# TuragaLab/flybody

Measured on AMD Instinct MI355X. Metric: env steps/sec (whole node), walk_imitation 4096-batch random-action rollout, higher is better.
Workload: dtype f64

## Files before the change

### flybody_amd/csrc/fb_constraint.hpp

```cpp
#pragma once
#include "fb_types.hpp"
#include "fb_math.hpp"
#include "fb_smooth.hpp"
#include "fb_newton.hpp"

#define JIDX(side, s, r) (((r)*2 + (side))*FB_MAXCH + (s))
#define MINIMP ((real)0.0001)
#define MAXIMP ((real)0.9999)

template <typename real>
FBD real get_impedance(const real* si, real pos, real margin) {
  real s0 = fmin(MAXIMP, fmax(MINIMP, si[0])), s1 = fmin(MAXIMP, fmax(MINIMP, si[1]));
  real s2 = fmax((real)0, si[2]), s3 = fmin(MAXIMP, fmax(MINIMP, si[3])), s4 = fmax((real)1, si[4]);
  if (s0 == s1 || s2 <= FB_MINV) return (real)0.5*(s0 + s1);
  real x = fabs((pos - margin)/s2);
  if (x >= 1) return s1;
  if (x <= 0) return s0;
  real y;
  if (s4 == 1) y = x;
  else if (s4 == 2) y = (x <= s3) ? x*x/s3 : 1 - (1 - x)*(1 - x)/(1 - s3);
  else if (x <= s3) y = pow(x, s4) / pow(s3, s4 - 1);
  else y = 1 - pow(1 - x, s4) / pow(1 - s3, s4 - 1);
  return s0 + y*(s1 - s0);
}
// ... 120 lines not shown
        real jp[3] = {0, 0, 0};
        const FB_LDS real* cp = w.lLD + 6*((sl < len) ? dof : 0);
        real cd[6];
#pragma unroll
        for (int k = 0; k < 6; k++) cd[k] = cp[k];
        if (sl < len) {
          real tt[3]; cross3(tt, cd, off);
          jp[0] = cd[3] + tt[0]; jp[1] = cd[4] + tt[1]; jp[2] = cd[5] + tt[2];
        }
        const real sgn = side ? (real)1 : (real)-1;
        for (int k = 0; k < cdim; k++) w.efc_J()[JIDX(side, sl, cadr + k)] = sgn*dot3(fr + 3*k, jp);
      }
    }
  }
  if (lane == 0) {
    if (nefc > w.istate()[IS_MAX_NEFC]) w.istate()[IS_MAX_NEFC] = nefc;
    if (nefc > 32) w.istate()[IS_N_GT32]++;
    if (nefc > 64) w.istate()[IS_N_GT64]++;
    w.istate()[IS_NEFC] = nefc; w.istate()[IS_NLIMIT] = nlimit; if (ob || nlimit > FB_MAXEFC_) { atomicOr(w.istate() + IS_WARN, (int)WARN_EFC_CAP); atomicOr(w.istate() + IS_WARN_EVER, (int)WARN_EFC_CAP); } }
  SYNC();
}

#define ARIDX(r, c) ((r)*((r) + 1)/2 + (c))

template <typename real, typename ARP>
FB_STAGE_B void d_build_AR(const DevModel<real>& M, const WS<real>& w, ARP AR, int nefc, int lane);

template <typename real>
FBD void project_row(const DevModel<real>& M, const WS<real>& w, int side, int r, int body, int len, const FB_LDS real* sd, real* y) {
  int chain[FB_MAXCH], rowadr[FB_MAXCH];
  load_chain(M, body, chain);
#pragma unroll
  for (int s = 0; s < FB_MAXCH; s++) { y[s] = (s < len) ? w.efc_J()[JIDX(side, s, r)] : (real)0; rowadr[s] = (int)w.lmadr()[chain[s]] + s; }
  const int chmax = M.chmax;
#pragma unroll
  for (int s = FB_MAXCH - 1; s >= 1; s--) {
    if (s < chmax) {
      const FB_LDS real* row = w.lLD + rowadr[s];
#pragma unroll
      for (int t = 0; t < s; t++) y[t] -= row[-t] * y[s];
    }
  }
#pragma unroll
  for (int s = 0; s < FB_MAXCH; s++) y[s] = (s < len) ? y[s]*sd[chain[s]] : (real)0;
}

template <int TRUNK, typename real, typename ARP>
FBD void ar_from_registers_t(const DevModel<real>& M, const WS<real>& w, ARP AR, int nefc, int lane, const real* yA, const real* yB, int bA, int bB, int lA, int lB) {
  const bool valid = lane < nefc;
  const int c = lane;
  const int* common = M.body_common; const int nb = M.nbody;
  int rbA = rdlane(bA, 0), rbB = rdlane(bB, 0);
  int cAA = common[rbA*nb + bA], cAB = common[rbA*nb + bB], cBA = common[rbB*nb + bA], cBB = common[rbB*nb + bB];
  const real Rc = valid ? w.efc_R()[c] : (real)0;
  real tr[TRUNK > 0 ? TRUNK : 1];
#pragma unroll
  for (int s = 0; s < TRUNK; s++) tr[s] = yA[s] + yB[s];
  for (int r = 0; r < nefc; r++) {
    int rlA = rdlane(lA, r), rlB = rdlane(lB, r);
    int cmAA = min(min(cAA, lA), rlA), cmAB = min(min(cAB, lB), rlA), cmBA = min(min(cBA, lA), rlB), cmBB = min(min(cBB, lB), rlB);
    if (r + 1 < nefc) {
      rbA = rdlane(bA, r + 1); rbB = rdlane(bB, r + 1);
      cAA = common[rbA*nb + bA]; cAB = common[rbA*nb + bB]; cBA = common[rbB*nb + bA]; cBB = common[rbB*nb + bB];
    }
    real acc = 0;
#pragma unroll
    for (int s = 0; s < TRUNK; s++) acc += rdlane(tr[s], r)*tr[s];
#pragma unroll
    for (int s0 = 0; s0 < FB_MAXCH; s0 += 4) {
      if (s0 + 4 > TRUNK && s0 < rlA) {
#pragma unroll
        for (int s = s0; s < s0 + 4; s++) if (s >= TRUNK) { real yr = rdlane(yA[s], r); if (s < cmAA) acc += yr*yA[s]; if (s < cmAB) acc += yr*yB[s]; }
      }
    }
#pragma unroll
    for (int s0 = 0; s0 < FB_MAXCH; s0 += 4) {
      if (s0 + 4 > TRUNK && s0 < rlB) {
#pragma unroll
        for (int s = s0; s < s0 + 4; s++) if (s >= TRUNK) { real yr = rdlane(yB[s], r); if (s < cmBA) acc += yr*yA[s]; if (s < cmBB) acc += yr*yB[s]; }
      }
    }
    if (valid && c <= r) {
      if (c == r) acc += Rc;
      AR[ARIDX(r, c)] = acc;
    }
  }
  SYNC();
}
template <int TRUNK, typename real, typename ARP>
FBD void ar_entry_lanes_t(const DevModel<real>& M, const WS<real>& w, ARP AR, int nefc, int lane, const real* yA, const real* yB, int bA, int bB, int lA, int lB) {
  const int* common = M.body_common; const int nb = M.nbody;
  const real Rl = w.efc_R()[lane];
  const int bodies = bA | (bB << 16), lens = lA | (lB << 8);
  real tr[TRUNK > 0 ? TRUNK : 1];
#pragma unroll
  for (int s = 0; s < TRUNK; s++) tr[s] = yA[s] + yB[s];
  unsigned any = 0;
#pragma unroll
  for (int g = 0; g < FB_MAXCH/4; g++) any |= (__ballot(lA > 4*g) != 0 ? 1u << g : 0u) | (__ballot(lB > 4*g) != 0 ? 0x100u << g : 0u);
  any = (unsigned)uniform_int((int)any);
  const int nent = nefc*(nefc + 1)/2;
  for (int p0 = 0; p0 < nent; p0 += FB_WAVE) {
    const int p = p0 + lane;
    const bool valid = p < nent;
    const int pp = valid ? p : 0;
    int r = (int)((sqrtf((float)(8*pp + 1)) - 1.0f)*0.5f);
    r -= (r*(r + 1)/2 > pp) ? 1 : 0;
    r += ((r + 1)*(r + 2)/2 <= pp) ? 1 : 0;
    const int c = pp - r*(r + 1)/2;
    const int rbod = nw_lane_i(bodies, r), cbod = nw_lane_i(bodies, c), rlen = nw_lane_i(lens, r), clen = nw_lane_i(lens, c);
    const int rbA = rbod & 0xffff, rbB = rbod >> 16, cbA = cbod & 0xffff, cbB = cbod >> 16;
    const int rlA = rlen & 0xff, rlB = rlen >> 8, clA = clen & 0xff, clB = clen >> 8;
    const int cmAA = min(min(common[rbA*nb + cbA], clA), rlA), cmAB = min(min(common[rbA*nb + cbB], clB), rlA);
    const int cmBA = min(min(common[rbB*nb + cbA], clA), rlB), cmBB = min(min(common[rbB*nb + cbB], clB), rlB);
    const real Rr = nw_lane(Rl, r);
    real acc = 0;
    {
      real tr_r[TRUNK > 0 ? TRUNK : 1], tr_c[TRUNK > 0 ? TRUNK : 1];
#pragma unroll
      for (int s = 0; s < TRUNK; s++) { tr_r[s] = nw_lane(tr[s], r); tr_c[s] = nw_lane(tr[s], c); }
#pragma unroll
      for (int s = 0; s < TRUNK; s++) acc += tr_r[s]*tr_c[s];
    }
#pragma unroll
    for (int s0 = 0; s0 < FB_MAXCH; s0 += 4) {
      if (s0 + 4 > TRUNK && ((any >> (s0/4)) & 1u)) {
        real yr[4], ya[4], yb[4];
#pragma unroll
        for (int s = s0; s < s0 + 4; s++) if (s >= TRUNK) { yr[s - s0] = nw_lane(yA[s], r); ya[s - s0] = nw_lane(yA[s], c); yb[s - s0] = nw_lane(yB[s], c); }
#pragma unroll
        for (int s = s0; s < s0 + 4; s++) if (s >= TRUNK) { if (s < cmAA) acc += yr[s - s0]*ya[s - s0]; if (s < cmAB) acc += yr[s - s0]*yb[s - s0]; }
      }
    }
#pragma unroll
    for (int s0 = 0; s0 < FB_MAXCH; s0 += 4) {
      if (s0 + 4 > TRUNK && ((any >> (8 + s0/4)) & 1u)) {
        real yr[4], ya[4], yb[4];
#pragma unroll
        for (int s = s0; s < s0 + 4; s++) if (s >= TRUNK) { yr[s - s0] = nw_lane(yB[s], r); ya[s - s0] = nw_lane(yA[s], c); yb[s - s0] = nw_lane(yB[s], c); }
#pragma unroll
        for (int s = s0; s < s0 + 4; s++) if (s >= TRUNK) { if (s < cmBA) acc += yr[s - s0]*ya[s - s0]; if (s < cmBB) acc += yr[s - s0]*yb[s - s0]; }
      }
    }
    if (valid) {
      if (c == r) acc += Rr;
      AR[p] = acc;
    }
  }
  SYNC();
}
template <typename real, typename ARP>
FBD void ar_from_registers(const DevModel<real>& M, const WS<real>& w, ARP AR, int nefc, int lane, const real* yA, const real* yB, int bA, int bB, int lA, int lB) {
  const bool entry = uniform_int(M.ar_entry_lanes) != 0;
  if (uniform_int(M.ntrunk) == FB_MAXTRUNK) {
    if (entry) ar_entry_lanes_t<FB_MAXTRUNK>(M, w, AR, nefc, lane, yA, yB, bA, bB, lA, lB);
    else ar_from_registers_t<FB_MAXTRUNK>(M, w, AR, nefc, lane, yA, yB, bA, bB, lA, lB);
  } else {
    if (entry) ar_entry_lanes_t<0>(M, w, AR, nefc, lane, yA, yB, bA, bB, lA, lB);
    else ar_from_registers_t<0>(M, w, AR, nefc, lane, yA, yB, bA, bB, lA, lB);
  }
}

template <typename real>
__device__ __forceinline__ void d_project_constraint(const DevModel<real>& M, const WS<real>& w, int lane) {
  int nefc = w.istate()[IS_NEFC];
  if (nefc == 0) return;
  FB_LDS real* sd = w.lx();
  for (int i = lane; i < M.nv; i += FB_WAVE) sd[i] = sqrt(w.lLD[w.lmadr()[i]]);
  SYNC();
  if (nefc <= FB_WAVE) {
    real yA[FB_MAXCH], yB[FB_MAXCH];
    int bA = 0, bB = 0, lA = 0, lB = 0;
    if (lane < nefc) { bA = w.efc_bA()[lane]; bB = w.efc_bB()[lane]; lA = w.efc_lA()[lane]; lB = w.efc_lB()[lane]; }
    project_row(M, w, 0, lane < nefc ? lane : 0, bA, lA, sd, yA);
    project_row(M, w, 1, lane < nefc ? lane : 0, bB, lB, sd, yB);
    if (nefc <= LdsCfg<real>::AR_ROWS) ar_from_registers(M, w, w.lAR(), nefc, lane, yA, yB, bA, bB, lA, lB);
    else ar_from_registers(M, w, w.AR(), nefc, lane, yA, yB, bA, bB, lA, lB);
    return;
  }
  for (int base = 0; base < nefc; base += FB_WAVE) {
    int r = base + lane;
    if (r < nefc) {
      for (int side = 0; side < 2; side++) {
        int body = side ? w.efc_bB()[r] : w.efc_bA()[r];
        int len = side ? w.efc_lB()[r] : w.efc_lA()[r];
        real y[FB_MAXCH];
        project_row(M, w, side, r, body, len, sd, y);
#pragma unroll
        for (int s = 0; s < FB_MAXCH; s++) w.efc_Y()[JIDX(side, s, r)] = y[s];
      }
    }
  }
  SYNC();
  const WS<real> wc = w;
  d_build_AR(M, wc, w.AR(), nefc, lane);
}

template <typename real, typename ARP>
FB_STAGE_B void d_build_AR(const DevModel<real>& M_, const WS<real>& w_, ARP AR, int nefc, int lane) {
  const DevModel<real>& M = as_constant(M_); const WS<real> w = ws_uniform(w_, M);
  for (int cbase = 0; cbase < nefc; cbase += FB_WAVE) {
    int c = cbase + lane;
    bool valid = c < nefc;
    real yA[FB_MAXCH], yB[FB_MAXCH];
    int bA = 0, bB = 0, lA = 0, lB = 0;
    if (valid) { bA = w.efc_bA()[c]; bB = w.efc_bB()[c]; lA = w.efc_lA()[c]; lB = w.efc_lB()[c]; }
#pragma unroll
    for (int s = 0; s < FB_MAXCH; s++) {
      yA[s] = valid ? w.efc_Y()[JIDX(0, s, c)] : (real)0;
      yB[s] = valid ? w.efc_Y()[JIDX(1, s, c)] : (real)0;
    }
    if (nefc <= FB_WAVE) {
      const int* common = M.body_common; const int nb = M.nbody;
      int rbA = rdlane(bA, 0), rbB = rdlane(bB, 0);
      int cAA = common[rbA*nb + bA], cAB = common[rbA*nb + bB], cBA = common[rbB*nb + bA], cBB = common[rbB*nb + bB];
      for (int r = 0; r < nefc; r++) {
        int rlA = rdlane(lA, r), rlB = rdlane(lB, r);
        int cmAA = min(min(cAA, lA), rlA), cmAB = min(min(cAB, lB), rlA), cmBA = min(min(cBA, lA), rlB), cmBB = min(min(cBB, lB), rlB);
        if (r + 1 < nefc) {
          rbA = rdlane(bA, r + 1); rbB = rdlane(bB, r + 1);
// ... 819 lines not shown
```

### flybody_amd/csrc/fb_engine.hip

```cpp
#ifdef FB_EMULATE
#include "emu/hip_emu.hpp"
#else
#include <hip/hip_runtime.h>
#endif
#include <algorithm>
#include <cmath>
#include <cstdio>
#include <cstdlib>
#include <cstring>
#include <map>
#include <stdexcept>
#include <string>
#include <vector>
#if defined(FB_EMULATE) && defined(FB_STATS)
extern "C" { long long fb_stats[64]; }
#endif

#include "../../include/flybody_engine.h"
#include "fb_step.hpp"
#include "fb_ik.hpp"
#include "fb_inverse.hpp"

static thread_local std::string g_err;
static int fail(const std::string& s) { g_err = s; return -1; }
// ... 853 lines not shown

static int alloc_obs(fb_batch* b, int nobs) {
  (void)hipFree(b->obs); b->obs = nullptr;
  HIPCHK(hipMalloc((void**)&b->obs, (size_t)b->n_env*nobs*sizeof(float)));
  HIPCHK(hipMemset(b->obs, 0, (size_t)b->n_env*nobs*sizeof(float)));
  b->nobs = nobs;
  return 0;
}

template <typename real>
static int build_devmodel(fb_batch* b, const fb_model* m, DevModel<real>& M) {
  memset(&M, 0, sizeof(M));
  M.nq = m->nq; M.nv = m->nv; M.nbody = m->nbody; M.njnt = m->njnt; M.ngeom = m->ngeom; M.nsite = m->nsite;
  M.nu = m->nu; M.na = m->na; M.ntendon = m->ntendon; M.npair = m->npair; M.nM = m->nM; M.nsubstep = m->nsubstep;
  M.nobsjnt = m->nobsjnt; M.napp = m->napp; M.nforce = m->nforce; M.ntouch = m->ntouch;
  M.site_thorax = m->i("sensor_site_thorax")[0]; M.nadh = (int)m->adh_act.size();
  M.iterations = m->i("opt_iterations")[0]; M.noslip_iterations = m->i("opt_noslip_iterations")[0];
  M.solver = (m->has("opt_solver", 1) && m->i("opt_solver")[0] == FB_SOLVER_PGS) ? FB_SOLVER_PGS : FB_SOLVER_NEWTON;
  M.timestep = (real)m->d("opt_timestep")[0]; M.control_timestep = (real)m->d("opt_control_timestep")[0];
  for (int k = 0; k < 3; k++) M.grav[k] = (real)m->d("opt_gravity")[k];
  M.density = (real)m->d("opt_density")[0]; M.viscosity = (real)m->d("opt_viscosity")[0];
  M.impratio = (real)m->d("opt_impratio")[0]; M.tolerance = (real)m->d("opt_tolerance")[0];
  {
    std::vector<double> rb; const double* r_ = m->d("geom_rbound");
    for (int g = 0; g < m->ngeom; g++) if (r_[g] > 0) rb.push_back(r_[g]);
    std::sort(rb.begin(), rb.end());
    M.vl_delta = (rb.empty() || m->npair <= 4*FB_WAVE) ? (real)0 : (real)(FB_VL_SCALE*rb[rb.size()/2]);
    { const char* e_ = getenv("FB_NO_NEIGHBOUR_LIST"); if (e_ && e_[0] == '1') M.vl_delta = 0; }
  }
  M.ar_entry_lanes = 1;
  { const char* e_ = getenv("FB_NO_AR_ENTRY_LANES"); if (e_ && e_[0] == '1') M.ar_entry_lanes = 0; }
  M.solver_handover = 1;
  { const char* e_ = getenv("FB_NO_SOLVER_HANDOVER"); if (e_ && e_[0] == '1') M.solver_handover = 0; }
  M.noslip_tolerance = (real)m->d("opt_noslip_tolerance")[0]; M.meaninertia = (real)m->d("stat_meaninertia")[0];
  M.totalmass = (real)m->totalmass;
  size_t c;
#define UI(field, name) { const int* s_ = m->i(name, &c); if (upload_i(b, s_, c, &M.field)) return -1; }
#define UV(field, vec) { if (upload_i(b, m->vec.data(), m->vec.size(), &M.field)) return -1; }
#define UD(field, name) { const double* s_ = m->d(name, &c); if (upload<real>(b, s_, c, &M.field)) return -1; }
  UI(body_parent, "body_parent") UI(body_dofadr, "body_dofadr")
  UV(body_nsub, body_nsub) UV(body_depth, body_depth) UV(body_chlen, body_chlen) UV(body_chain, body_chain) UV(body_common, body_common)
  UI(jnt_type, "jnt_type") UI(jnt_qposadr, "jnt_qposadr") UI(jnt_dofadr, "jnt_dofadr") UI(jnt_bodyid, "jnt_bodyid") UI(jnt_limited, "jnt_limited")
  UI(dof_bodyid, "dof_bodyid") UI(dof_jntid, "dof_jntid") UI(dof_Madr, "dof_Madr") UV(dof_depth, dof_depth)
  UV(dof_ndesc, dof_ndesc) UV(body_fluid_geom, body_fluid_geom) UV(sens_body, sens_body) M.nsensbody = (int)m->sens_body.size();
  UV(dof_jump, dof_jump) UV(dof_vbef, dof_vbef) UV(body_veldof, body_veldof)
  UV(dof_cl, dof_cl) UV(dof_gen, dof_gen) UV(gen_k, gen_k) UV(gen_m, gen_m) UV(fwd_tab, fwd_tab) UV(fwd_pack, fwd_pack) UV(fac_w, fac_w) UV(fac_band, fac_band) UV(fac_dof, fac_dof) M.ntrunk = m->ntrunk; M.prefix_split = m->prefix_split;
  { int dmax = 0, d2 = 1 << 20; for (int bq = 1; bq < m->nbody; bq++) { dmax = std::max(dmax, m->body_depth[bq]); if (bq >= FB_WAVE) d2 = std::min(d2, m->body_depth[bq]); } M.fk_dmax = dmax; M.fk2_dlo = d2; }
  { int cm = 0; for (int bq = 0; bq < m->nbody; bq++) cm = std::max(cm, m->body_chlen[bq]); M.chmax = cm; }
  {
    std::vector<int> second(FB_WAVE, -1);
    bool ok = m->nbody > FB_WAVE && m->nbody <= 2*FB_WAVE && getenv("FB_NO_FK_MERGE") == nullptr;
    for (int bq = FB_WAVE; ok && bq < m->nbody; bq++) {
      int pick = -1;
      for (int l = 0; l < FB_WAVE && pick < 0; l++) if (second[l] < 0 && (l == 0 || m->body_depth[l] < m->body_depth[bq])) pick = l;
      if (pick < 0) ok = false; else second[pick] = bq;
    }
    M.fk_second = nullptr;
    if (ok && upload_i(b, second.data(), second.size(), &M.fk_second)) return -1;
  }
  UI(wing_act_idx, "wing_action_idx")
  if (m->has("leg_joints", 1)) { UI(leg_jnt, "leg_joints") M.nlegjnt = (int)c; for (size_t k = 0; k < c; k++) if (m->i("leg_joints")[k] < 0 || m->i("leg_joints")[k] >= m->njnt) return fail("fb_batch_create: leg_joints out of range"); }
  else { UV(leg_jnt, adh_act) M.nlegjnt = 0; }
  M.task = m->task_id; M.user_idx = m->i("user_action_idx")[0]; M.nact = m->nu + (M.user_idx >= 0 ? 1 : 0);
  for (int k = 0; k < 3; k++) M.com_offset[k] = (real)m->d("com_offset")[k];
  M.nlevel = m->nlevel;
  UI(geom_type, "geom_type") UI(geom_bodyid, "geom_bodyid") UI(site_bodyid, "site_bodyid") UI(site_type, "site_type")
// ... 582 lines not shown
    case FB_QM: *f = {REAL_ARENA, o.qM, (size_t)m->nM}; break;
    case FB_EFC_FORCE: *f = {REAL_ARENA, o.efc_force, FB_MAXEFC_}; break;
    case FB_QFRC_ACTUATOR: *f = {REAL_ARENA, o.qfrc_actuator, (size_t)m->nv}; break;
    case FB_QFRC_CONSTRAINT: *f = {REAL_ARENA, o.qfrc_constraint, (size_t)m->nv}; break;
    case FB_SUBTREE_COM: *f = {REAL_ARENA, o.com, 3}; break;
    case FB_NCON: *f = {INT_ARENA, o.istate + IS_NCON, 1}; break;
    case FB_NEFC: *f = {INT_ARENA, o.istate + IS_NEFC, 1}; break;
    case FB_SOLVER_NITER: *f = {INT_ARENA, o.istate + IS_NITER, 1}; break;
    case FB_STEP_COUNT: *f = {INT_ARENA, o.istate + IS_STEP, 1}; break;
    case FB_PROF: *f = {INT_ARENA, o.prof, 2*FB_NPROF}; break;
    case FB_REWARD_FACTORS: *f = {REAL_ARENA, o.rfac, 5}; break;
    case FB_GEOM_XPOS: *f = {REAL_ARENA, o.gxpos, (size_t)3*m->ngeom}; break;
    case FB_GEOM_XMAT: *f = {REAL_ARENA, o.gxmat, (size_t)9*m->ngeom}; break;
    case FB_CVEL: *f = {REAL_ARENA, o.cvel, (size_t)6*m->nbody}; break;
    case FB_OBS: *f = {F32_ARRAY, 0, (size_t)b->nobs, b->obs, no_ref}; break;
    case FB_REWARD: *f = {F32_ARRAY, 0, 1, b->reward}; break;
    case FB_DISCOUNT: *f = {F32_ARRAY, 0, 1, b->discount}; break;
    case FB_STEP_TYPE: *f = {I32_ARRAY, 0, 1, b->step_type}; break;
    case FB_WARN: *f = {INT_ARENA, o.istate + IS_WARN, 1}; break;
    case FB_WARN_EVER: *f = {INT_ARENA, o.istate + IS_WARN_EVER, 1}; break;
    case FB_SIZE_STATS: *f = {INT_ARENA, o.istate + IS_MAX_NCON, 4}; break;
    case FB_STEP_TICKS: *f = {I32_ARRAY, 0, 1, b->cost}; break;
    case FB_LAUNCH_ORDER: *f = {I32_ARRAY, 0, 1, b->order}; break;
    case FB_SITE_XPOS: *f = {REAL_ARENA, o.sxpos, (size_t)3*m->nsite}; break;
    case FB_IK_ERR: *f = {F64_ARRAY, 0, 2, b->ik_err, no_ik}; break;
    case FB_IK_STEPS: *f = {I32_ARRAY, 0, 2, b->ik_steps, no_ik}; break;
    case FB_QFRC_INVERSE: *f = {F64_ARRAY, 0, (size_t)m->nv, b->inv_qfrc, no_inv}; break;
    case FB_CONTACT_FORCE: *f = {F64_ARRAY, 0, (size_t)3*FB_MAXCON_, b->inv_cforce, no_inv}; break;
    case FB_QFRC_APPLIED: *f = {REAL_ARRAY, 0, (size_t)m->nv, b->qfrc_applied, no_frc}; break;
    case FB_XFRC_APPLIED: *f = {REAL_ARRAY, 0, (size_t)6*m->nbody, b->xfrc_applied, no_frc}; break;
    case FB_ENV_MODEL: *f = {I32_ARRAY, 0, 1, b->env_model, no_grp}; break;
    case FB_QFRC_LAW: *f = {REAL_ARRAY, 0, (size_t)m->nv, b->law_out, "fb_batch_get: no control law (fb_batch_set_control_law sets one)"}; break;
    case FB_CONTROL_LAW: return fail("FB_CONTROL_LAW is [n_rows][5][nv], not one row per environment: read and write it through fb_batch_device_ptr, set it with fb_batch_set_control_law");
    default: return fail("unknown field");
  }
  return 0;
}

static int alloc_forces(fb_batch* b) {
  if (b->qfrc_applied && b->xfrc_applied) return 0;
  const size_t rs = real_size(b);
  HIPCHK(hipDeviceSynchronize());
  void *q = nullptr, *x = nullptr;
  const size_t nq_ = (size_t)b->n_env*b->m->nv*rs, nx_ = (size_t)b->n_env*6*b->m->nbody*rs;
  if (hipMalloc(&q, nq_) != hipSuccess || hipMalloc(&x, nx_) != hipSuccess || hipMemset(q, 0, nq_) != hipSuccess || hipMemset(x, 0, nx_) != hipSuccess) {
    (void)hipFree(q); (void)hipFree(x); (void)hipGetLastError();
    return fail("applied forces: device allocation failed");
  }
  HIPCHK(hipDeviceSynchronize());
  b->qfrc_applied = q; b->xfrc_applied = x;
  return 0;
}

extern "C" int fb_batch_clear_forces(fb_batch* b) {
  if (!b) return fail("fb_batch_clear_forces: null batch");
  if (b->law_coef) return fail("fb_batch_clear_forces: a control law is set, and its kernel (k_step_law) reads the force arrays; call fb_batch_set_control_law(batch, NULL) first");
  HIPCHK(hipSetDevice(b->device));
  HIPCHK(hipDeviceSynchronize());
  (void)hipFree(b->qfrc_applied); (void)hipFree(b->xfrc_applied);
  b->qfrc_applied = b->xfrc_applied = nullptr;
  return 0;
}

extern "C" int fb_batch_forces_active(const fb_batch* b) {
  if (!b) return fail("fb_batch_forces_active: null batch");
  return b->qfrc_applied ? 1 : 0;
// ... 253 lines not shown
```

### flybody_amd/csrc/fb_math.hpp

```cpp
#pragma once
#ifdef FB_EMULATE
#include "emu/hip_emu.hpp"
#else
#include <hip/hip_runtime.h>
#endif

#define FBD __device__ __forceinline__
#ifdef FB_EMULATE
#define FB_NOINLINE
#else
#define FB_NOINLINE __attribute__((noinline))
#endif
#define FB_STAGE_A __device__ __forceinline__
#define FB_STAGE_B __device__ FB_NOINLINE
#define FB_STAGE_FS __device__ FB_NOINLINE
#define FB_MINV ((real)1e-15)

#ifndef FB_EMULATE
#define FB_DIV_STEPS 2
#define FB_RSQ_STEPS 1
#define FB_INV_STEPS 2
FBD double fb_div(double a, double b) {
  double r = __builtin_amdgcn_rcp(b);
#pragma unroll
// ... 193 lines not shown
  int lo = __builtin_amdgcn_update_dpp(0, __double2loint(v), CTRL, 0xf, 0xf, true);
  int hi = __builtin_amdgcn_update_dpp(0, __double2hiint(v), CTRL, 0xf, 0xf, true);
  return __hiloint2double(hi, lo);
}
template <typename real> FBD real wave_sum(real v) {
  v += dpp_mov<0xB1>(v);
  v += dpp_mov<0x4E>(v);
  v += dpp_mov<0x141>(v);
  v += dpp_mov<0x140>(v);
  return (rdlane(v, 0) + rdlane(v, 16)) + (rdlane(v, 32) + rdlane(v, 48));
}
#endif
#ifdef FB_EMULATE
template <typename real> FBD real wave_sum_lo(real v, bool) { return wave_sum(v); }
#else
template <typename real> FBD real wave_sum_lo(real v, bool row0) {
  v += dpp_mov<0xB1>(v); v += dpp_mov<0x4E>(v); v += dpp_mov<0x141>(v); v += dpp_mov<0x140>(v);
  real r = rdlane(v, 0);
  if (!row0) r = (r + rdlane(v, 16)) + (rdlane(v, 32) + rdlane(v, 48));
  return r;
}
#endif
#ifdef FB_EMULATE
template <typename real> FBD real quad_sum(real v) { v += shfl_xor_r(v, 1); v += shfl_xor_r(v, 2); return v; }
#else
template <typename real> FBD real quad_sum(real v) { v += dpp_mov<0xB1>(v); v += dpp_mov<0x4E>(v); return v; }
#endif
FBD double shfl_xor_any(double v, int m) { return __shfl_xor(v, m, 64); }
FBD float shfl_xor_any(float v, int m) { return __shfl_xor(v, m, 64); }
FBD int wave_sum_i(int v) {
  for (int m = 32; m >= 1; m >>= 1) v += __shfl_xor(v, m, 64);
  return v;
}
FBD int wave_excl_scan(int v, int lane) {
  int s = v;
  for (int d = 1; d < 64; d <<= 1) { int t = __shfl_up(s, d, 64); if (lane >= d) s += t; }
  return s - v;
}
```

### flybody_amd/csrc/fb_types.hpp

```cpp
#pragma once
#ifdef FB_EMULATE
#include "emu/hip_emu.hpp"
#else
#include <hip/hip_runtime.h>
#endif
#include <stdint.h>

#if defined(FB_EMULATE) && defined(FB_STATS)
extern "C" { extern long long fb_stats[64]; }
#define FB_STAT(k) (fb_stats[k]++)
#else
#define FB_STAT(k) do {} while (0)
#endif

#define FB_WAVE 64
#define FB_EPB 4
#define FB_MAXCH 20
#define FB_MAXGEN 16
#define FB_LDS_SCRATCH 1216
#define FB_LGEN 6
#define FB_BODYREC 40
#define FB_MAXTRUNK 6
#define FB_FSLOT 18
#define FB_FGEN 2
// ... 47 lines not shown
  X(qpos, M.nq) X(qvel, M.nv) X(act, M.na + 1) X(ctrl, M.nu) X(qacc, M.nv) X(qacc_ws, M.nv) X(act_dot, M.na + 1) \
  X(sens, FB_NSENS) X(sens_acc, FB_NSENS) X(simtime, 1) X(wbfreq, 1) X(dsshift, 2) X(rfac, 6) \
  X(xpos, 3*M.nbody) X(xquat, 4*M.nbody)  \
  X(xaxis, 3*M.njnt)  X(gxpos, 3*M.ngeom) X(gxmat, 9*M.ngeom) X(sxpos, 3*M.nsite) X(sxmat, 9*M.nsite) X(com, 4) \
  X(cinert, 10*M.nbody) X(cdof, 6*M.nv) X(cvel, 6*M.nbody) \
  X(qM, M.nM) X(qLD, M.nM) \
  X(qfrc_bias, M.nv) X(qfrc_passive, M.nv) X(qfrc_actuator, M.nv) X(qfrc_smooth, M.nv) X(qacc_smooth, M.nv) \
  X(qfrc_constraint, M.nv) X(ten_length, M.ntendon + 1) X(act_force, M.nu) \
  X(con_dist, FB_MAXCON_) X(con_pos, 3*FB_MAXCON_) X(con_frame, 9*FB_MAXCON_) \
  X(efc_J, 2*FB_MAXCH*FB_MAXEFC_) \
  X(efc_pos, FB_MAXEFC_) X(efc_margin, FB_MAXEFC_) X(efc_R, FB_MAXEFC_) X(efc_D, FB_MAXEFC_) X(efc_K, FB_MAXEFC_) \
  X(efc_B, FB_MAXEFC_) X(efc_imp, FB_MAXEFC_) X(efc_aref, FB_MAXEFC_) X(efc_b, FB_MAXEFC_) X(efc_force, FB_MAXEFC_) \
  X(efc_vel, FB_MAXEFC_) X(efc_mu, FB_MAXEFC_) X(efc_jar, FB_MAXEFC_) X(efc_s1, FB_MAXEFC_) X(efc_s2, FB_MAXEFC_)  \
  X(cacc, 6*M.nbody) X(cfrc, 6*M.nbody) X(cfrc_ext, 6*M.nbody) X(cabias, 6*M.nbody) \
   \
  X(efc_Y, 2*FB_MAXCH*FB_MAXEFC_) X(AR, FB_MAXEFC_*(FB_MAXEFC_ + 1))  \
  X(nws, FB_NWS_VECS*FB_MAXEFC_)  \
  X(vl_pos, 3*M.ngeom)

#define FB_WS_INT(X) \
  X(istate, IS_N) X(prof, 2*FB_NPROF) X(con_pair, FB_MAXCON_) X(con_efc, FB_MAXCON_) X(con_dim, FB_MAXCON_) X(cand, 2*FB_MAXCON_ + 64) \
  X(efc_type, FB_MAXEFC_) X(efc_id, FB_MAXEFC_) X(efc_bA, FB_MAXEFC_) X(efc_bB, FB_MAXEFC_) X(efc_lA, FB_MAXEFC_) X(efc_lB, FB_MAXEFC_) \
  X(efc_k, FB_MAXEFC_)  X(efc_eA, FB_MAXEFC_) X(efc_eB, FB_MAXEFC_)  \
  X(vl_list, FB_VLMAX)

struct WSOff {
#define X(name, n) uint32_t name;
  FB_WS_REAL(X)
  FB_WS_INT(X)
#undef X
  uint32_t nreal, nint;
};

template <typename real>
struct DevModel {
  int nq, nv, nbody, njnt, ngeom, nsite, nu, na, ntendon, npair, nM, nsubstep;
  int nobsjnt, napp, nforce, ntouch, site_thorax, nadh;
  int iterations, noslip_iterations, solver;
  real timestep, control_timestep, grav[3], density, viscosity, impratio, tolerance, noslip_tolerance, meaninertia, totalmass;
  real vl_delta;
  int ar_entry_lanes;
  int solver_handover;
  GP<const int> body_parent, body_dofadr, body_nsub, body_depth;
  GP<const int> body_chlen;
  GP<const int> body_chain;
  GP<const int> body_common;
  GP<const int> jnt_type, jnt_qposadr, jnt_dofadr, jnt_bodyid, jnt_limited;
  GP<const int> dof_bodyid, dof_jntid, dof_Madr, dof_depth;
  GP<const int> dof_ndesc;
  int nlevel;
  GP<const int> dof_cl;
  GP<const int> dof_gen;
  GP<const int> gen_k, gen_m;
  GP<const int> fwd_tab;
  GP<const int> fwd_pack;
  GP<const int> fac_w;
  GP<const int> fac_band;
  GP<const int> fac_dof;
  int ntrunk;
  int prefix_split;
  int chmax;
  int fk_dmax, fk2_dlo;
  const int* fk_second;
  GP<const int> geom_type, geom_bodyid, site_bodyid, site_type;
  GP<const int> tendon_adr, tendon_num;
  GP<const int> act_trntype, act_trnid, act_dyntype, act_biastype, act_ctrllimited, act_forcelimited, act_actadr;
  GP<const int> adh_act;
  GP<const int> wrap_qadr;
  GP<const int> act_wn, act_wdof, act_lenadr;
  GP<const real> act_wcoef;
  GP<const int> action_to_ctrl;
  GP<const int> pair_geom1, pair_geom2, pair_condim;
  GP<const int> pair_body;
  GP<const int> pair_word;
  GP<const int> plane_geoms; int nplane;
  GP<const int> obs_jnt, app_sites, force_sites, touch_sites, wing_jnt;
  GP<const int> dof_jump;
  GP<const int> dof_vbef;
  GP<const int> body_veldof;
  GP<const int> sens_body; int nsensbody;
  GP<const real> body_mass, body_inertia, body_invweight0, body_box;
  GP<const real> body_rec;
  GP<const real> jnt_axis, jnt_stiffness, jnt_range, jnt_solref, jnt_solimp, jnt_margin;
// ... 70 lines not shown
```

### flybody_amd/engine.py

```python
from __future__ import annotations

import collections
import ctypes as C
import os
from typing import Dict, Optional

import numpy as np

from .model_blob import load_npz, pack_model

_HERE = os.path.dirname(os.path.abspath(__file__))
HIP_LIB = os.path.join(_HERE, 'libflybody_hip.so')
HIP_LIB_DENSE = os.path.join(_HERE, 'libflybody_hip_dense.so')
ASSETS = os.path.join(_HERE, 'assets')

MAXCON, MAXEFC, NSENSOR = 64, 192, 33
_F64, _F32, _I32 = np.float64, np.float32, np.int32
FIELDS = dict(
    QPOS=(0, _F64, 'nq'), QVEL=(1, _F64, 'nv'), ACT=(2, _F64, 'na'), CTRL=(3, _F64, 'nu'), QACC=(4, _F64, 'nv'),
    XPOS=(5, _F64, (3, 'nbody')), XQUAT=(6, _F64, (4, 'nbody')), SENSORDATA=(7, _F64, NSENSOR), OBS=(8, _F32, 'nobs'),
    REWARD=(9, _F32, 1), DISCOUNT=(10, _F32, 1), STEP_TYPE=(11, _I32, 1), NCON=(12, _I32, 1), NEFC=(13, _I32, 1),
    SOLVER_NITER=(14, _I32, 1), QFRC_BIAS=(15, _F64, 'nv'), QFRC_PASSIVE=(16, _F64, 'nv'), QACC_SMOOTH=(17, _F64, 'nv'),
    QM=(18, _F64, 'nM'), CONTACT=(19, _F64, MAXCON*8), EFC_FORCE=(20, _F64, MAXEFC), QFRC_ACTUATOR=(21, _F64, 'nv'),
    QFRC_CONSTRAINT=(22, _F64, 'nv'), STEP_COUNT=(23, _I32, 1), SUBTREE_COM=(24, _F64, 3), PROF=(25, _I32, 112),
    REWARD_FACTORS=(26, _F64, 5), GEOM_XPOS=(27, _F64, (3, 'ngeom')), GEOM_XMAT=(28, _F64, (9, 'ngeom')), CVEL=(29, _F64, (6, 'nbody')),
    STEP_TICKS=(30, _I32, 1), LAUNCH_ORDER=(31, _I32, 1), WARN=(32, _I32, 1), WARN_EVER=(33, _I32, 1), SIZE_STATS=(34, _I32, 4),
    SITE_XPOS=(35, _F64, (3, 'nsite')), IK_ERR=(36, _F64, 2), IK_STEPS=(37, _I32, 2), QFRC_INVERSE=(38, _F64, 'nv'),
    CONTACT_FORCE=(39, _F64, 3*MAXCON), QFRC_APPLIED=(40, _F64, 'nv'), XFRC_APPLIED=(41, _F64, (6, 'nbody')), ENV_MODEL=(42, _I32, 1),
    QFRC_LAW=(43, _F64, 'nv'), CONTROL_LAW=(44, _F64, (5, 'nv')))
TASK_IDS = dict(walk_imitation=0, flight_imitation=1, walk_on_ball=2, template_task=3)
LAW_ROWS = ('bias', 'act_gain', 'pos_gain', 'pos_ref', 'vel_gain')
WARN_BITS = dict(CONTACT_CAP=1, EFC_CAP=2, SOLVER_MAXITER=4, CCD_MAXITER=8, SCHED_WAIT=16, SOLVER_FALLBACK=32, MODEL_ID=64)

ST = dict(ACT=0, ACC_PRE=1, SOLVE=2, ACC_SOLVE=3, ACC_POST=4, CONSTR_A=5, CONSTR_B=6, SENS=7, EULER_PRE=8, FACTOR=9, EULER_SOLVE=10,
          EULER_POST=11, KIN=12, COLL=13, SUBEND=14, PRE=32, POST=33)


def stage_sequence(nsubstep: int):
    DAMP, HALF, P = 1 << 8, 1 << 9, lambda m: m << 12
    sub = [('actuation', ST['ACT']), ('smooth_rhs', ST['ACC_PRE']), ('factor_M', ST['FACTOR']), ('solve_smooth', ST['SOLVE'] | HALF),
           ('qacc_smooth_copy', ST['ACC_POST'] | P(1)), ('project_constraint', ST['ACC_POST'] | P(2)), ('constraint_solve', ST['CONSTR_A']),
           ('solve_constraint', ST['SOLVE']), ('qacc', ST['CONSTR_B']), ('sensor_acc', ST['SENS']), ('euler_rhs', ST['EULER_PRE']),
           ('factor_M_hD', ST['FACTOR'] | DAMP), ('solve_euler', ST['SOLVE'] | HALF), ('integrate', ST['EULER_POST']),
           ('kinematics', ST['KIN'] | P(1)), ('com_pos', ST['KIN'] | P(2)), ('crb', ST['KIN'] | P(4)), ('collision', ST['COLL'] | P(1)),
           ('make_constraint', ST['COLL'] | P(2)), ('velocity', ST['COLL'] | P(4)), ('substep_end', ST['SUBEND'])]
    return [('task_pre', ST['PRE'])] + sub*nsubstep + [('task_post', ST['POST'])]


_libs: Dict[str, C.CDLL] = {}


class EngineError(RuntimeError):
    pass


def load_library(lib_path: Optional[str] = None) -> C.CDLL:
    path = lib_path or HIP_LIB
    if path in _libs:
        return _libs[path]
    if not os.path.exists(path):
        raise EngineError(f'{path} not found: build it with `python -c "import __graft_entry__ as g; g.build()"` '
                          '(hipcc --offload-arch=gfx950); there is no CPU fallback')
# ... 371 lines not shown
```

### include/flybody_engine.h

```cpp
#ifndef FLYBODY_ENGINE_H
#define FLYBODY_ENGINE_H
#include <stddef.h>
#include <stdint.h>

#ifdef __cplusplus
extern "C" {
#endif

typedef struct fb_model fb_model;
typedef struct fb_batch fb_batch;

enum {
  FB_QPOS = 0,
  FB_QVEL = 1,
  FB_ACT = 2,
  FB_CTRL = 3,
  FB_QACC = 4,
  FB_XPOS = 5,
  FB_XQUAT = 6,
  FB_SENSORDATA = 7,
  FB_OBS = 8,
  FB_REWARD = 9,
  FB_DISCOUNT = 10,
  FB_STEP_TYPE = 11,
  FB_NCON = 12,
  FB_NEFC = 13,
  FB_SOLVER_NITER = 14,
  FB_QFRC_BIAS = 15,
  FB_QFRC_PASSIVE = 16,
  FB_QACC_SMOOTH = 17,
  FB_QM = 18,
  FB_CONTACT = 19,
  FB_EFC_FORCE = 20,
  FB_QFRC_ACTUATOR = 21,
  FB_QFRC_CONSTRAINT = 22,
  FB_STEP_COUNT = 23,
  FB_SUBTREE_COM = 24,
  FB_GEOM_XPOS = 27,
  FB_GEOM_XMAT = 28,
  FB_CVEL = 29,
  FB_STEP_TICKS = 30,
  FB_LAUNCH_ORDER = 31,
  FB_REWARD_FACTORS = 26,
  FB_PROF = 25,
  FB_WARN = 32,
  FB_WARN_EVER = 33,
  FB_SIZE_STATS = 34,
  FB_SITE_XPOS = 35,
  FB_IK_ERR = 36,
  FB_IK_STEPS = 37,
  FB_QFRC_INVERSE = 38,
  FB_CONTACT_FORCE = 39,
  FB_QFRC_APPLIED = 40,
  FB_XFRC_APPLIED = 41,
  FB_ENV_MODEL = 42,
  FB_QFRC_LAW = 43,
  FB_CONTROL_LAW = 44,
  FB_NFIELD
};

enum { FB_MAXCON = 64, FB_MAXEFC = 192, FB_NSENSOR = 33 };
enum { FB_WARN_CONTACT_CAP = 1, FB_WARN_EFC_CAP = 2, FB_WARN_SOLVER_MAXITER = 4, FB_WARN_CCD_MAXITER = 8,
       FB_WARN_SOLVER_FALLBACK = 32 ,
       FB_WARN_SCHED_WAIT = 16 ,
       FB_WARN_MODEL_ID = 64  };

int fb_model_dim(const fb_model* m, const char* name);

int fb_model_load(const void* blob, size_t nbytes, fb_model** out);
void fb_model_destroy(fb_model* m);

int fb_batch_create(const fb_model* m, int n_env, int device, int precision, fb_batch** out);
void fb_batch_destroy(fb_batch* b);

int fb_batch_set_reference(fb_batch* b, const double* ref_qpos, const double* ref_qvel, int T,
                           int future_steps, double terminal_com_dist, double time_limit);

int fb_batch_set_time_limit(fb_batch* b, double time_limit);

int fb_batch_set_wbpg(fb_batch* b, const double* traj, const double* phase, const int32_t* offset, const double* freqs,
                      int nfreq, double base_freq, double rel_range, double rate, uint32_t seed);

typedef struct fb_walk_dataset {
  int32_t n_traj, n_joints, n_sites, n_select;
  const int32_t* traj_offset;
  const double* qpos;
  const double* qvel;
  const double* root2site;
  const double* joint_quat;
  const int32_t* joint_ids;
// ... 75 lines not shown
```

Baseline: 869,600.

## Project constraint rows with paired half-waves and bound chain loop by wave max length

When there are at most 32 constraint rows, each half of the wave projects one side of every row, so a single project_row call replaces the two per-lane calls. The Delassus entry-lane kernel gains a PAIRED template variant that fetches the B side from lane+32 through shuffles. Separately, the back-substitution loop in project_row is capped at the wave's maximum chain length instead of the model-wide maximum. The change also adds an FB_DELASSUS readback field, environment toggles, and an explicit SGPR clobber in f64 dense builds, which may affect register allocation.

```diff
diff --git a/flybody_amd/csrc/fb_constraint.hpp b/flybody_amd/csrc/fb_constraint.hpp
--- a/flybody_amd/csrc/fb_constraint.hpp
+++ b/flybody_amd/csrc/fb_constraint.hpp
@@ -176,7 +176,8 @@
   load_chain(M, body, chain);
 #pragma unroll
   for (int s = 0; s < FB_MAXCH; s++) { y[s] = (s < len) ? w.efc_J()[JIDX(side, s, r)] : (real)0; rowadr[s] = (int)w.lmadr()[chain[s]] + s; }
-  const int chmax = M.chmax;
+  int chmax = M.chmax;
+  if (uniform_int(M.project_paired) & FB_PM_BOUND) chmax = min(chmax, wave_max_i(len));
 #pragma unroll
   for (int s = FB_MAXCH - 1; s >= 1; s--) {
     if (s < chmax) {
@@ -231,17 +232,24 @@
   }
   SYNC();
 }
-template <int TRUNK, typename real, typename ARP>
+template <int TRUNK, bool PAIRED, typename real, typename ARP>
 FBD void ar_entry_lanes_t(const DevModel<real>& M, const WS<real>& w, ARP AR, int nefc, int lane, const real* yA, const real* yB, int bA, int bB, int lA, int lB) {
   const int* common = M.body_common; const int nb = M.nbody;
+  constexpr int OB = PAIRED ? 32 : 0;
   const real Rl = w.efc_R()[lane];
-  const int bodies = bA | (bB << 16), lens = lA | (lB << 8);
+  const int bodies = PAIRED ? (bA | (lA << 16)) : (bA | (bB << 16)), lens = lA | (lB << 8);
   real tr[TRUNK > 0 ? TRUNK : 1];
 #pragma unroll
-  for (int s = 0; s < TRUNK; s++) tr[s] = yA[s] + yB[s];
+  for (int s = 0; s < TRUNK; s++) {
+    if (PAIRED) { const real o = __shfl(yA[s], lane ^ 32, 64); tr[s] = (lane & 32) ? o + yA[s] : yA[s] + o; }
+    else tr[s] = yA[s] + yB[s];
+  }
   unsigned any = 0;
 #pragma unroll
-  for (int g = 0; g < FB_MAXCH/4; g++) any |= (__ballot(lA > 4*g) != 0 ? 1u << g : 0u) | (__ballot(lB > 4*g) != 0 ? 0x100u << g : 0u);
+  for (int g = 0; g < FB_MAXCH/4; g++) {
+    if (PAIRED) { const unsigned long long m = __ballot(lA > 4*g); any |= ((unsigned)m != 0 ? 1u << g : 0u) | ((unsigned)(m >> 32) != 0 ? 0x100u << g : 0u); }
+    else any |= (__ballot(lA > 4*g) != 0 ? 1u << g : 0u) | (__ballot(lB > 4*g) != 0 ? 0x100u << g : 0u);
+  }
   any = (unsigned)uniform_int((int)any);
   const int nent = nefc*(nefc + 1)/2;
   for (int p0 = 0; p0 < nent; p0 += FB_WAVE) {
@@ -252,9 +260,9 @@
     r -= (r*(r + 1)/2 > pp) ? 1 : 0;
     r += ((r + 1)*(r + 2)/2 <= pp) ? 1 : 0;
     const int c = pp - r*(r + 1)/2;
-    const int rbod = nw_lane_i(bodies, r), cbod = nw_lane_i(bodies, c), rlen = nw_lane_i(lens, r), clen = nw_lane_i(lens, c);
-    const int rbA = rbod & 0xffff, rbB = rbod >> 16, cbA = cbod & 0xffff, cbB = cbod >> 16;
-    const int rlA = rlen & 0xff, rlB = rlen >> 8, clA = clen & 0xff, clB = clen >> 8;
+    const int f0 = nw_lane_i(bodies, r), f1 = nw_lane_i(bodies, c), f2 = nw_lane_i(PAIRED ? bodies : lens, PAIRED ? OB + r : r), f3 = nw_lane_i(PAIRED ? bodies : lens, PAIRED ? OB + c : c);
+    const int rbA = f0 & 0xffff, rbB = PAIRED ? f2 & 0xffff : f0 >> 16, cbA = f1 & 0xffff, cbB = PAIRED ? f3 & 0xffff : f1 >> 16;
+    const int rlA = PAIRED ? f0 >> 16 : f2 & 0xff, rlB = PAIRED ? f2 >> 16 : f2 >> 8, clA = PAIRED ? f1 >> 16 : f3 & 0xff, clB = PAIRED ? f3 >> 16 : f3 >> 8;
     const int cmAA = min(min(common[rbA*nb + cbA], clA), rlA), cmAB = min(min(common[rbA*nb + cbB], clB), rlA);
     const int cmBA = min(min(common[rbB*nb + cbA], clA), rlB), cmBB = min(min(common[rbB*nb + cbB], clB), rlB);
     const real Rr = nw_lane(Rl, r);
@@ -271,7 +279,7 @@
       if (s0 + 4 > TRUNK && ((any >> (s0/4)) & 1u)) {
         real yr[4], ya[4], yb[4];
 #pragma unroll
-        for (int s = s0; s < s0 + 4; s++) if (s >= TRUNK) { yr[s - s0] = nw_lane(yA[s], r); ya[s - s0] = nw_lane(yA[s], c); yb[s - s0] = nw_lane(yB[s], c); }
+        for (int s = s0; s < s0 + 4; s++) if (s >= TRUNK) { yr[s - s0] = nw_lane(yA[s], r); ya[s - s0] = nw_lane(yA[s], c); yb[s - s0] = nw_lane(yB[s], OB + c); }
 #pragma unroll
         for (int s = s0; s < s0 + 4; s++) if (s >= TRUNK) { if (s < cmAA) acc += yr[s - s0]*ya[s - s0]; if (s < cmAB) acc += yr[s - s0]*yb[s - s0]; }
       }
@@ -281,7 +289,7 @@
       if (s0 + 4 > TRUNK && ((any >> (8 + s0/4)) & 1u)) {
         real yr[4], ya[4], yb[4];
 #pragma unroll
-        for (int s = s0; s < s0 + 4; s++) if (s >= TRUNK) { yr[s - s0] = nw_lane(yB[s], r); ya[s - s0] = nw_lane(yA[s], c); yb[s - s0] = nw_lane(yB[s], c); }
+        for (int s = s0; s < s0 + 4; s++) if (s >= TRUNK) { yr[s - s0] = nw_lane(yB[s], OB + r); ya[s - s0] = nw_lane(yA[s], c); yb[s - s0] = nw_lane(yB[s], OB + c); }
 #pragma unroll
         for (int s = s0; s < s0 + 4; s++) if (s >= TRUNK) { if (s < cmBA) acc += yr[s - s0]*ya[s - s0]; if (s < cmBB) acc += yr[s - s0]*yb[s - s0]; }
       }
@@ -297,21 +305,48 @@
 FBD void ar_from_registers(const DevModel<real>& M, const WS<real>& w, ARP AR, int nefc, int lane, const real* yA, const real* yB, int bA, int bB, int lA, int lB) {
   const bool entry = uniform_int(M.ar_entry_lanes) != 0;
   if (uniform_int(M.ntrunk) == FB_MAXTRUNK) {
-    if (entry) ar_entry_lanes_t<FB_MAXTRUNK>(M, w, AR, nefc, lane, yA, yB, bA, bB, lA, lB);
+    if (entry) ar_entry_lanes_t<FB_MAXTRUNK, false>(M, w, AR, nefc, lane, yA, yB, bA, bB, lA, lB);
     else ar_from_registers_t<FB_MAXTRUNK>(M, w, AR, nefc, lane, yA, yB, bA, bB, lA, lB);
   } else {
-    if (entry) ar_entry_lanes_t<0>(M, w, AR, nefc, lane, yA, yB, bA, bB, lA, lB);
+    if (entry) ar_entry_lanes_t<0, false>(M, w, AR, nefc, lane, yA, yB, bA, bB, lA, lB);
     else ar_from_registers_t<0>(M, w, AR, nefc, lane, yA, yB, bA, bB, lA, lB);
   }
+}
+
+template <typename real, typename ARP>
+FBD void ar_from_paired(const DevModel<real>& M, const WS<real>& w, ARP AR, int nefc, int lane, const real* y, int body, int len) {
+  if (uniform_int(M.ntrunk) == FB_MAXTRUNK) ar_entry_lanes_t<FB_MAXTRUNK, true>(M, w, AR, nefc, lane, y, y, body, body, len, len);
+  else ar_entry_lanes_t<0, true>(M, w, AR, nefc, lane, y, y, body, body, len, len);
+}
+
+template <typename real>
+FBD void ar_publish(const WS<real>& w, int nefc, int lane) {
+#ifdef FB_EMULATE
+  if (nefc <= LdsCfg<real>::AR_ROWS) { for (int p = lane; p < nefc*(nefc + 1)/2; p += FB_WAVE) w.AR()[p] = w.lAR()[p]; }
+#endif
 }
 
 template <typename real>
 __device__ __forceinline__ void d_project_constraint(const DevModel<real>& M, const WS<real>& w, int lane) {
+#if FB_F64_DENSE && !defined(FB_EMULATE)
+  asm volatile("" ::: "s53", "s54", "s55", "s64", "s65", "s66", "s67", "s68", "s69", "s70", "s71", "s80", "s81", "s82", "s83", "s84", "s85", "s86", "s87",
+               "s96", "s97", "s98", "s99");
+#endif
   int nefc = w.istate()[IS_NEFC];
   if (nefc == 0) return;
   FB_LDS real* sd = w.lx();
   for (int i = lane; i < M.nv; i += FB_WAVE) sd[i] = sqrt(w.lLD[w.lmadr()[i]]);
   SYNC();
+  if (nefc <= 32 && (uniform_int(M.project_paired) & FB_PM_PAIRED) && uniform_int(M.ar_entry_lanes) != 0) {
+    real y[FB_MAXCH];
+    const int row = min(lane & 31, nefc - 1), side = lane >> 5;
+    const int body = (side ? w.efc_bB() : w.efc_bA())[row], len = (side ? w.efc_lB() : w.efc_lA())[row];
+    project_row(M, w, side, row, body, len, sd, y);
+    if (nefc <= LdsCfg<real>::AR_ROWS) ar_from_paired(M, w, w.lAR(), nefc, lane, y, body, len);
+    else ar_from_paired(M, w, w.AR(), nefc, lane, y, body, len);
+    ar_publish(w, nefc, lane);
+    return;
+  }
   if (nefc <= FB_WAVE) {
     real yA[FB_MAXCH], yB[FB_MAXCH];
     int bA = 0, bB = 0, lA = 0, lB = 0;
@@ -320,16 +355,17 @@
     project_row(M, w, 1, lane < nefc ? lane : 0, bB, lB, sd, yB);
     if (nefc <= LdsCfg<real>::AR_ROWS) ar_from_registers(M, w, w.lAR(), nefc, lane, yA, yB, bA, bB, lA, lB);
     else ar_from_registers(M, w, w.AR(), nefc, lane, yA, yB, bA, bB, lA, lB);
+    ar_publish(w, nefc, lane);
     return;
   }
   for (int base = 0; base < nefc; base += FB_WAVE) {
-    int r = base + lane;
-    if (r < nefc) {
-      for (int side = 0; side < 2; side++) {
-        int body = side ? w.efc_bB()[r] : w.efc_bA()[r];
-        int len = side ? w.efc_lB()[r] : w.efc_lA()[r];
-        real y[FB_MAXCH];
-        project_row(M, w, side, r, body, len, sd, y);
+    const int r = base + lane; const bool valid = r < nefc; const int rr = valid ? r : 0;
+    for (int side = 0; side < 2; side++) {
+      const int body = valid ? (side ? w.efc_bB()[rr] : w.efc_bA()[rr]) : 0;
+      const int len = valid ? (side ? w.efc_lB()[rr] : w.efc_lA()[rr]) : 0;
+      real y[FB_MAXCH];
+      project_row(M, w, side, rr, body, len, sd, y);
+      if (valid) {
 #pragma unroll
         for (int s = 0; s < FB_MAXCH; s++) w.efc_Y()[JIDX(side, s, r)] = y[s];
       }
diff --git a/flybody_amd/csrc/fb_engine.hip b/flybody_amd/csrc/fb_engine.hip
--- a/flybody_amd/csrc/fb_engine.hip
+++ b/flybody_amd/csrc/fb_engine.hip
@@ -909,6 +909,8 @@
   { const char* e_ = getenv("FB_NO_AR_ENTRY_LANES"); if (e_ && e_[0] == '1') M.ar_entry_lanes = 0; }
   M.solver_handover = 1;
   { const char* e_ = getenv("FB_NO_SOLVER_HANDOVER"); if (e_ && e_[0] == '1') M.solver_handover = 0; }
+  M.project_paired = FB_PM_PAIRED | FB_PM_BOUND;
+  { const char* e_ = getenv("FB_NO_PROJECT_PAIRED"); if (e_) { if (e_[0] == '1') M.project_paired = 0; else if (e_[0] == '2') M.project_paired = FB_PM_BOUND; else if (e_[0] == '3') M.project_paired = FB_PM_PAIRED; } }
   M.noslip_tolerance = (real)m->d("opt_noslip_tolerance")[0]; M.meaninertia = (real)m->d("stat_meaninertia")[0];
   M.totalmass = (real)m->totalmass;
   size_t c;
@@ -1557,6 +1559,7 @@
     case FB_ENV_MODEL: *f = {I32_ARRAY, 0, 1, b->env_model, no_grp}; break;
     case FB_QFRC_LAW: *f = {REAL_ARRAY, 0, (size_t)m->nv, b->law_out, "fb_batch_get: no control law (fb_batch_set_control_law sets one)"}; break;
     case FB_CONTROL_LAW: return fail("FB_CONTROL_LAW is [n_rows][5][nv], not one row per environment: read and write it through fb_batch_device_ptr, set it with fb_batch_set_control_law");
+    case FB_DELASSUS: *f = {REAL_ARENA, o.AR, (size_t)FB_MAXEFC_*(FB_MAXEFC_ + 1)/2}; break;
     default: return fail("unknown field");
   }
   return 0;
diff --git a/flybody_amd/csrc/fb_math.hpp b/flybody_amd/csrc/fb_math.hpp
--- a/flybody_amd/csrc/fb_math.hpp
+++ b/flybody_amd/csrc/fb_math.hpp
@@ -249,6 +249,10 @@
   for (int m = 32; m >= 1; m >>= 1) v += __shfl_xor(v, m, 64);
   return v;
 }
+FBD int wave_max_i(int v) {
+  for (int m = 32; m >= 1; m >>= 1) { const int t = __shfl_xor(v, m, 64); v = t > v ? t : v; }
+  return uniform_int(v);
+}
 FBD int wave_excl_scan(int v, int lane) {
   int s = v;
   for (int d = 1; d < 64; d <<= 1) { int t = __shfl_up(s, d, 64); if (lane >= d) s += t; }
diff --git a/flybody_amd/csrc/fb_types.hpp b/flybody_amd/csrc/fb_types.hpp
--- a/flybody_amd/csrc/fb_types.hpp
+++ b/flybody_amd/csrc/fb_types.hpp
@@ -103,6 +103,8 @@
   uint32_t nreal, nint;
 };
 
+#define FB_PM_PAIRED 1
+#define FB_PM_BOUND 2
 template <typename real>
 struct DevModel {
   int nq, nv, nbody, njnt, ngeom, nsite, nu, na, ntendon, npair, nM, nsubstep;
@@ -120,6 +122,7 @@
   GP<const int> dof_bodyid, dof_jntid, dof_Madr, dof_depth;
   GP<const int> dof_ndesc;
   int nlevel;
+  int project_paired;
   GP<const int> dof_cl;
   GP<const int> dof_gen;
   GP<const int> gen_k, gen_m;
diff --git a/flybody_amd/engine.py b/flybody_amd/engine.py
--- a/flybody_amd/engine.py
+++ b/flybody_amd/engine.py
@@ -27,7 +27,7 @@
     STEP_TICKS=(30, _I32, 1), LAUNCH_ORDER=(31, _I32, 1), WARN=(32, _I32, 1), WARN_EVER=(33, _I32, 1), SIZE_STATS=(34, _I32, 4),
     SITE_XPOS=(35, _F64, (3, 'nsite')), IK_ERR=(36, _F64, 2), IK_STEPS=(37, _I32, 2), QFRC_INVERSE=(38, _F64, 'nv'),
     CONTACT_FORCE=(39, _F64, 3*MAXCON), QFRC_APPLIED=(40, _F64, 'nv'), XFRC_APPLIED=(41, _F64, (6, 'nbody')), ENV_MODEL=(42, _I32, 1),
-    QFRC_LAW=(43, _F64, 'nv'), CONTROL_LAW=(44, _F64, (5, 'nv')))
+    QFRC_LAW=(43, _F64, 'nv'), CONTROL_LAW=(44, _F64, (5, 'nv')), DELASSUS=(45, _F64, MAXEFC*(MAXEFC + 1)//2))
 TASK_IDS = dict(walk_imitation=0, flight_imitation=1, walk_on_ball=2, template_task=3)
 LAW_ROWS = ('bias', 'act_gain', 'pos_gain', 'pos_ref', 'vel_gain')
 WARN_BITS = dict(CONTACT_CAP=1, EFC_CAP=2, SOLVER_MAXITER=4, CCD_MAXITER=8, SCHED_WAIT=16, SOLVER_FALLBACK=32, MODEL_ID=64)
diff --git a/include/flybody_engine.h b/include/flybody_engine.h
--- a/include/flybody_engine.h
+++ b/include/flybody_engine.h
@@ -56,6 +56,7 @@
   FB_ENV_MODEL = 42,
   FB_QFRC_LAW = 43,
   FB_CONTROL_LAW = 44,
+  FB_DELASSUS = 45,
   FB_NFIELD
 };
 
```

New measurement: 874,600 (median of 6 runs). Within noise of the previous version (+0.6%).
